# yshen47/SGAM_NeurIPS22

Measured on AMD Instinct MI355X. Metric: generated RGB-D frames/sec (256x256, GoogleEarth), higher is better.
Workload: dtype f32; 1 GPU; GoogleEarth-Infinite 256x256 inference loop (BASELINE configs[2]): forward-splat warp (N<=3) + VQGAN encode/quantise(4096)/decode + frame feedback, in-HBM frame store; frames_per_gpu=1105, scenes=1, parallelism=scene-parallel x1, launch=hip-graph replay of the VQGAN forward, f32_products=exact hi/lo fp16 split on the fp16 matrix cores, fp32 accumulate

## Files before the change

sgam_neurips22_amd/build.py:

```python
import hashlib
import os
import shutil
import subprocess
import sys

PKG = os.path.dirname(os.path.abspath(__file__))
CSRC = os.path.join(PKG, "csrc")
LIBDIR = os.environ.get("SGAM_LIB_DIR") or os.path.join(PKG, "lib")
LIB = os.path.join(LIBDIR, "libsgam_hip.so")
ARCH = "gfx950"

SOURCES = {
    "conv_gemm.hip": [],
    "norm_softmax.hip": [],
    "groupnorm.hip": [],
    "h16.hip": [],
    "conv_f32x.hip": [],
    "h16_halo.hip": [],
    "attention.hip": [],
    "vq.hip": ["-ffp-contract=off"],
    "layout.hip": ["-ffp-contract=off"],
    "warp.hip": ["-ffp-contract=off"],
    "gemm_gn_f32x.hip": [],
    "train.hip": [],
    "eval.hip": ["-ffp-contract=off"],
    "kmeans.hip": ["-ffp-contract=off"],
    "imageio.hip": ["-ffp-contract=off"],
    "build_info.hip": [],
    "tsdf.hip": ["-ffp-contract=off"],
    "mesh_raster.hip": ["-ffp-contract=off"],
    "point_raster.hip": ["-ffp-contract=off"],
    "point_nn.hip": ["-ffp-contract=off"],
    "point_cloud.hip": ["-ffp-contract=off"],
    "point_icp.hip": ["-ffp-contract=off"],
    "point_global.hip": ["-ffp-contract=off"],
    "mesh_ops.hip": ["-ffp-contract=off"],
    "mesh_query.hip": ["-ffp-contract=off"],
    "mesh_ray.hip": ["-ffp-contract=off"],
    "mesh_bvh.hip": ["-ffp-contract=off"],
    "inception.hip": ["-ffp-contract=off"],
    "feature_metrics.hip": ["-ffp-contract=off"],
}
COMMON = ["-O3", "-std=c++17", "-fPIC", f"--offload-arch={ARCH}", "-Wall", "-Wno-unused-function"]


def _hipcc():
    for cand in (os.environ.get("HIPCC"), shutil.which("hipcc"), "/opt/rocm/bin/hipcc"):
        if cand and os.path.exists(cand):
            return cand
    raise RuntimeError("hipcc not found: libsgam_hip.so cannot be built (ROCm toolchain required)")


def _git(*args):
    try:
        r = subprocess.run(["git", "-C", os.path.join(PKG, "..")] + list(args), capture_output=True, text=True, timeout=10)
        return r.stdout.strip() if r.returncode == 0 else None
    except (OSError, subprocess.SubprocessError):
        return None


_STAMP_PATHS = ["sgam_neurips22_amd/csrc", "include", "sgam_neurips22_amd/build.py"]


def build_stamp(headers):
    srcs = sorted(os.path.join(CSRC, f) for f in SOURCES if os.path.exists(os.path.join(CSRC, f)) and f != "build_info.hip")
    digest = _digest(srcs + headers, [COMMON] + [SOURCES[os.path.basename(p)] for p in srcs])[:12]
    stamp_file = os.path.join(LIBDIR, "BUILD_STAMP")
    commit = _git("log", "-1", "--format=%h", "--abbrev=12", "--", *_STAMP_PATHS)
    if commit:
        if _git("status", "--porcelain", "--", *_STAMP_PATHS):
            commit += "+dirty"
    else:
        commit = "nogit"
        if os.path.exists(stamp_file):
            old = open(stamp_file).read().split()
            if len(old) == 2 and old[1] == digest:
                commit = old[0]
    return commit, digest, stamp_file


def _digest(paths, flags):
    h = hashlib.sha256()
    for p in sorted(paths, key=os.path.basename):
        h.update(os.path.basename(p).encode())
        with open(p, "rb") as f:
            h.update(f.read())
    h.update(repr(flags).encode())
    return h.hexdigest()


def build(force=False, verbose=False):
    hipcc = _hipcc()
    os.makedirs(LIBDIR, exist_ok=True)
    headers = [os.path.join(CSRC, f) for f in os.listdir(CSRC) if f.endswith(".h")]
    headers.append(os.path.join(PKG, "..", "include", "sgam_hip.h"))
    objs, relink = [], force or not os.path.exists(LIB)
    commit, digest, stamp_file = build_stamp(headers)
    SOURCES["build_info.hip"] = [f'-DSGAM_BUILD_COMMIT="{commit}"', f'-DSGAM_BUILD_DIGEST="{digest}"']
    for src, extra in SOURCES.items():
        path = os.path.join(CSRC, src)
        if not os.path.exists(path):
            continue
        obj = os.path.join(LIBDIR, src.replace(".hip", ".o"))
        stamp = obj + ".sha"
        dig = _digest([path] + headers, COMMON + extra)
        old = open(stamp).read() if os.path.exists(stamp) else ""
        if force or not os.path.exists(obj) or old != dig:
            cmd = [hipcc] + COMMON + extra + ["-c", path, "-o", obj]
            if verbose:
                print(" ".join(cmd), flush=True)
            subprocess.check_call(cmd)
            with open(stamp, "w") as f:
                f.write(dig)
            relink = True
        objs.append(obj)
    if relink:
        cmd = [hipcc, "-shared", "-fPIC", f"--offload-arch={ARCH}", "-o", LIB] + objs
        if verbose:
            print(" ".join(cmd), flush=True)
        subprocess.check_call(cmd)
    with open(stamp_file, "w") as f:
        f.write(f"{commit} {digest}\n")
    return LIB


if __name__ == "__main__":
    print(build(force="--force" in sys.argv, verbose=True))
```

sgam_neurips22_amd/csrc/attention.hip:

```cpp
#include "sgam_common.h"

namespace {

typedef unsigned int u32x4 __attribute__((ext_vector_type(4)));
typedef unsigned int u32x2 __attribute__((ext_vector_type(2)));
typedef _Float16 f16x8 __attribute__((ext_vector_type(8)));

constexpr int AD = 256;
constexpr int KB = 32;
constexpr int BLK_BYTES = KB * AD * 4;
constexpr float P_LIFT = 10.0f;
constexpr float LOG2E = 1.4426950408889634f;
constexpr float RESCALE_TAU = 5.0f;

__device__ __forceinline__ f32x16 mfma16(u32x4 a, u32x4 b, f32x16 c) {
    return __builtin_amdgcn_mfma_f32_32x32x16_f16(__builtin_bit_cast(f16x8, a), __builtin_bit_cast(f16x8, b), c, 0, 0, 0);
}

__device__ __forceinline__ void split8(const float *v, u32x4 &hi, u32x4 &lo) {
#pragma unroll
    for (int e = 0; e < 4; ++e) {
        const _Float16 h0 = (_Float16)v[2 * e], h1 = (_Float16)v[2 * e + 1];
        const _Float16 l0 = (_Float16)(v[2 * e] - (float)h0), l1 = (_Float16)(v[2 * e + 1] - (float)h1);
        hi[e] = (unsigned)__builtin_bit_cast(unsigned short, h0) | ((unsigned)__builtin_bit_cast(unsigned short, h1) << 16);
        lo[e] = (unsigned)__builtin_bit_cast(unsigned short, l0) | ((unsigned)__builtin_bit_cast(unsigned short, l1) << 16);
    }
}

__global__ __launch_bounds__(256) void attn_split_kv_kernel(const float *__restrict__ k, const float *__restrict__ v, int ld,
                                                            int n, unsigned short *__restrict__ kf,
                                                            unsigned short *__restrict__ vf) {
    const int gid = blockIdx.x * 256 + threadIdx.x;
    const int row = gid & 31, h = (gid >> 5) & 1, t = (gid >> 6) & 1, tile = (gid >> 7) & 7, kb = gid >> 10;
    if (kb * KB >= n) return;
    float kv[8], vv[8];
    const float *kp = k + (int64_t)(kb * KB + row) * ld + tile * 32 + t * 16 + h * 8;
    const f32x4 k0 = *reinterpret_cast<const f32x4 *>(kp), k1 = *reinterpret_cast<const f32x4 *>(kp + 4);
#pragma unroll
    for (int e = 0; e < 4; ++e) {
        kv[e] = k0[e];
        kv[4 + e] = k1[e];
    }
#pragma unroll
    for (int s = 0; s < 8; ++s) {
        const int key = 4 * h + 8 * (2 * t + (s >> 2)) + (s & 3);
        vv[s] = v[(int64_t)(kb * KB + key) * ld + tile * 32 + row];
    }
    u32x4 hi, lo;
    const int64_t piece = ((int64_t)(kb * 8 + tile) * 256 + (t * 2 + h) * 32 + row) * 8;
    split8(kv, hi, lo);
    *reinterpret_cast<u32x4 *>(kf + piece) = hi;
    *reinterpret_cast<u32x4 *>(kf + piece + 128 * 8) = lo;
    split8(vv, hi, lo);
    *reinterpret_cast<u32x4 *>(vf + piece) = hi;
    *reinterpret_cast<u32x4 *>(vf + piece + 128 * 8) = lo;
}

struct AttnParams {
    const unsigned short *qf;
    const float *q;
    const unsigned short *kf, *vf;
    float *ws_o;
    float *ws_ml;
    int ld, n, blocks_per_split;
    int n_img, nsplit;
    float qscale;
};

constexpr int NSPLIT = 8;

typedef __attribute__((address_space(1))) const void gptr_t;
typedef __attribute__((address_space(3))) void lptr_t;

__global__ __launch_bounds__(256) void attn_flash_f32x_kernel(const AttnParams p) {
    __shared__ __attribute__((aligned(16))) unsigned char smem[4 * BLK_BYTES];
    const int tid = threadIdx.x, lane = tid & 63, wave = tid >> 6;
    const int sp = blockIdx.x % p.nsplit, qb = blockIdx.x / p.nsplit;
    const int q0 = qb * 128 + wave * 32;
    const int lq = lane & 31, lh = lane >> 5;
    const int kb0 = ((qb * 128) / p.n_img) * (p.n_img / KB) + sp * p.blocks_per_split, kb1 = kb0 + p.blocks_per_split;
    const unsigned char *kg = reinterpret_cast<const unsigned char *>(p.kf), *vg = reinterpret_cast<const unsigned char *>(p.vf);

    const int wave_s = __builtin_amdgcn_readfirstlane(wave);
    auto dma1 = [&](const unsigned char *g, int kb, int slot, const int i) {
        const unsigned char *src = g + (int64_t)kb * BLK_BYTES + wave_s * 8192 + (i >> 2) * 4096 + lane * 16;
        unsigned char *dst = smem + slot * BLK_BYTES + wave_s * 8192 + (i >> 2) * 4096;
        switch (i & 3) {
        case 0: __builtin_amdgcn_global_load_lds((gptr_t *)src, (lptr_t *)dst, 16, 0, 0); break;
        case 1: __builtin_amdgcn_global_load_lds((gptr_t *)src, (lptr_t *)dst, 16, 1024, 0); break;
        case 2: __builtin_amdgcn_global_load_lds((gptr_t *)src, (lptr_t *)dst, 16, 2048, 0); break;
        default: __builtin_amdgcn_global_load_lds((gptr_t *)src, (lptr_t *)dst, 16, 3072, 0); break;
        }
    };
    auto dma = [&](const unsigned char *g, int kb, int slot) {
#pragma unroll
        for (int i = 0; i < 8; ++i) dma1(g, kb, slot, i);
    };
    u32x4 qh[16], ql[16];
    if (p.qf) {
        const unsigned short *qb = p.qf + (int64_t)(q0 >> 5) * (16 * 1024) + lane * 8;
#pragma unroll
        for (int t = 0; t < 16; ++t) {
            qh[t] = *reinterpret_cast<const u32x4 *>(qb + t * 1024);
            ql[t] = *reinterpret_cast<const u32x4 *>(qb + t * 1024 + 512);
        }
    } else {
        const float *qp = p.q + (int64_t)(q0 + lq) * p.ld + lh * 8;
#pragma unroll
        for (int t = 0; t < 16; ++t) {
            const f32x4 a = *reinterpret_cast<const f32x4 *>(qp + t * 16), b = *reinterpret_cast<const f32x4 *>(qp + t * 16 + 4);
            float v[8];
#pragma unroll
            for (int e = 0; e < 4; ++e) {
                v[e] = a[e] * p.qscale;
                v[4 + e] = b[e] * p.qscale;
            }
            split8(v, qh[t], ql[t]);
        }
    }

    f32x16 o[8];
#pragma unroll
    for (int i = 0; i < 8; ++i)
#pragma unroll
        for (int e = 0; e < 16; ++e) o[i][e] = 0.f;
    float m_run = -INFINITY, l_run = 0.f;

    const int nb = kb1 - kb0;
    auto blk = [&](int j) { return kb0 + (j < nb ? j : nb - 1); };
    dma(kg, blk(0), 0);
    dma(vg, blk(0), 2);
    dma(kg, blk(1), 1);

    u32x4 fh[3], fl[3];
    f32x16 sacc[2];
    float s[16], pe[2];
    u32x4 ph[2], pl[2];
    auto lds_off = [](const unsigned char *ptr) {
        return (unsigned)(uintptr_t)(__attribute__((address_space(3))) const unsigned char *)ptr;
    };
#define ATTN_DS_READ(dst, addr, off) asm volatile("ds_read_b128 %0, %1 offset:%2" : "=v"(dst) : "v"(addr), "i"(off))
#define ATTN_DS_WAIT(n, set) asm volatile("s_waitcnt lgkmcnt(" #n ")" : "+v"(fh[set]), "+v"(fl[set]))
#define ATTN_BARRIER(cnt)                                        \
    do {                                                          \
        asm volatile("s_waitcnt vmcnt(" #cnt ")" ::: "memory");   \
        __builtin_amdgcn_s_barrier();                             \
    } while (0)
    auto smfma = [&](const int t) {
        sacc[(3 * t) & 1] = mfma16(fh[t % 3], qh[t], sacc[(3 * t) & 1]);
        sacc[(3 * t + 1) & 1] = mfma16(fh[t % 3], ql[t], sacc[(3 * t + 1) & 1]);
        sacc[(3 * t + 2) & 1] = mfma16(fl[t % 3], qh[t], sacc[(3 * t + 2) & 1]);
    };
#define ATTN_FRAG(set, base, t)                                              \
    do {                                                                      \
        ATTN_DS_READ(fh[set], base, ((t) >> 1) * 4096 + ((t) & 1) * 1024);        \
        ATTN_DS_READ(fl[set], base, ((t) >> 1) * 4096 + (2 + ((t) & 1)) * 1024);  \
    } while (0)
    ATTN_BARRIER(0);

    {
        const unsigned lk = lds_off(smem + lane * 16);
#pragma unroll
        for (int e = 0; e < 16; ++e) sacc[0][e] = sacc[1][e] = 0.f;
        ATTN_FRAG(0, lk, 0);
        ATTN_FRAG(1, lk, 1);
#pragma unroll
        for (int t = 0; t < 16; ++t) {
            if (t + 2 < 16) ATTN_FRAG((t + 2) % 3, lk, t + 2);
            if (t + 2 < 16) ATTN_DS_WAIT(4, t % 3);
            else if (t + 1 < 16) ATTN_DS_WAIT(2, t % 3);
            else ATTN_DS_WAIT(0, t % 3);
            smfma(t);
        }
        float mloc = -INFINITY;
#pragma unroll
        for (int e = 0; e < 16; ++e) {
            s[e] = (sacc[0][e] + sacc[1][e]) * LOG2E;
            mloc = fmaxf(mloc, s[e]);
        }
        m_run = fmaxf(mloc, __shfl_xor(mloc, 32, 64));
        ATTN_BARRIER(0);
        dma(kg, blk(2), 0);
    }

    for (int j = 0; j < nb; ++j) {
        const int buf = j & 1;
        const unsigned lk = lds_off(smem + (buf ^ 1) * BLK_BYTES + lane * 16);
        const unsigned lv = lds_off(smem + (2 + buf) * BLK_BYTES + lane * 16);
        const int kb_k = blk(j + 3), kb_v = blk(j + 1);
#pragma unroll
        for (int e = 0; e < 16; ++e) sacc[0][e] = sacc[1][e] = 0.f;
        ATTN_FRAG(0, lk, 0);
        ATTN_FRAG(1, lk, 1);
#pragma unroll
        for (int t = 0; t < 16; ++t) {
            if (t + 2 < 16) ATTN_FRAG((t + 2) % 3, lk, t + 2);
            if (t < 8) dma1(vg, kb_v, 2 + (buf ^ 1), t);
            if (t + 2 < 16) ATTN_DS_WAIT(4, t % 3);
            else if (t + 1 < 16) ATTN_DS_WAIT(2, t % 3);
            else ATTN_DS_WAIT(0, t % 3);
            smfma(t);
            pe[t & 1] = __builtin_amdgcn_exp2f(s[t] - m_run + P_LIFT);
            l_run += pe[t & 1];
            if (t & 1) {
                typedef _Float16 f16x2 __attribute__((ext_vector_type(2)));
                const f16x2 h = __builtin_bit_cast(f16x2, __builtin_amdgcn_cvt_pkrtz(pe[0], pe[1]));
                const f16x2 l = __builtin_bit_cast(f16x2, __builtin_amdgcn_cvt_pkrtz(pe[0] - (float)h[0], pe[1] - (float)h[1]));
                ph[t >> 3][(t & 7) >> 1] = __builtin_bit_cast(unsigned, h);
                pl[t >> 3][(t & 7) >> 1] = __builtin_bit_cast(unsigned, l);
            }
        }
        ATTN_BARRIER(16);
        float mloc = -INFINITY;
        ATTN_FRAG(16 % 3, lv, 0);
        ATTN_FRAG(17 % 3, lv, 1);
#pragma unroll
        for (int u = 0; u < 16; ++u) {
            if (u + 2 < 16) ATTN_FRAG((16 + u + 2) % 3, lv, u + 2);
            if (u < 8) dma1(kg, kb_k, buf ^ 1, u);
            if (u + 2 < 16) ATTN_DS_WAIT(4, (16 + u) % 3);
            else if (u + 1 < 16) ATTN_DS_WAIT(2, (16 + u) % 3);
            else ATTN_DS_WAIT(0, (16 + u) % 3);
            const int i = u >> 1, t = u & 1, set = (16 + u) % 3;
            o[i] = mfma16(fh[set], ph[t], o[i]);
            o[i] = mfma16(fh[set], pl[t], o[i]);
            o[i] = mfma16(fl[set], ph[t], o[i]);
            if (u >= 4) {
#pragma unroll
                for (int e = (u - 4) * 4 / 3; e < (u - 3) * 4 / 3; ++e) {
                    s[e] = (sacc[0][e] + sacc[1][e]) * LOG2E;
                    mloc = fmaxf(mloc, s[e]);
                }
            }
        }
        if (j + 1 < nb) {
            mloc = fmaxf(mloc, __shfl_xor(mloc, 32, 64));
            const float m_new = fmaxf(m_run, mloc);
            if (__any(m_new > m_run + RESCALE_TAU)) {
                const float alpha = __builtin_amdgcn_exp2f(m_run - m_new);
                l_run *= alpha;
#pragma unroll
                for (int i = 0; i < 8; ++i)
#pragma unroll
                    for (int e = 0; e < 16; ++e) {
                        float x = o[i][e], tmp;
                        asm volatile("v_accvgpr_read_b32 %1, %0\n\tv_mul_f32 %1, %1, %2\n\tv_accvgpr_write_b32 %0, %1"
                                     : "+a"(x), "=&v"(tmp)
                                     : "v"(alpha));
                        o[i][e] = x;
                    }
                m_run = m_new;
            }
        }
        ATTN_BARRIER(16);
    }
#undef ATTN_FRAG
#undef ATTN_BARRIER
#undef ATTN_DS_WAIT
#undef ATTN_DS_READ

    l_run += __shfl_xor(l_run, 32, 64);
    if (lh == 0) {
        float *ml = p.ws_ml + ((int64_t)sp * p.n + q0 + lq) * 2;
        ml[0] = m_run;
        ml[1] = l_run;
    }
    float *wo = p.ws_o + ((int64_t)sp * (p.n / 32) + (q0 >> 5)) * (AD * 32) + lq;
#pragma unroll
    for (int i = 0; i < 8; ++i)
#pragma unroll
        for (int e = 0; e < 16; ++e)
            wo[(32 * i + 8 * (e >> 2) + 4 * lh + (e & 3)) * 32] = o[i][e];
    asm volatile("s_waitcnt vmcnt(0)" ::: "memory");
}

template <int NS>
__global__ __launch_bounds__(256) void attn_combine_kernel(const float *__restrict__ ws_o, const float *__restrict__ ws_ml,
                                                           float *__restrict__ out, int ldo, int n, int32_t *range_flag) {
    __shared__ float tile[32][33];
    const int qt = blockIdx.x >> 3, dg = blockIdx.x & 7;
    const int q = threadIdx.x & 31, dsub = threadIdx.x >> 5;
    float w[NS], l[NS], o[NS][4], M = -INFINITY, L = 0.f;
#pragma unroll
    for (int s = 0; s < NS; ++s) {
        const float *ml = ws_ml + ((int64_t)s * n + qt * 32 + q) * 2;
        w[s] = ml[0];
        l[s] = ml[1];
    }
#pragma unroll
    for (int s = 0; s < NS; ++s)
#pragma unroll
        for (int j = 0; j < 4; ++j) o[s][j] = ws_o[(((int64_t)s * (n / 32) + qt) * AD + dg * 32 + dsub * 4 + j) * 32 + q];
#pragma unroll
    for (int s = 0; s < NS; ++s) M = fmaxf(M, w[s]);
#pragma unroll
    for (int s = 0; s < NS; ++s) {
        w[s] = __builtin_amdgcn_exp2f(w[s] - M);
        L += w[s] * l[s];
    }
    const float inv = 1.0f / L;
    float acc[4] = {0.f, 0.f, 0.f, 0.f};
#pragma unroll
    for (int s = 0; s < NS; ++s)
#pragma unroll
        for (int j = 0; j < 4; ++j) acc[j] += w[s] * o[s][j];
#pragma unroll
    for (int j = 0; j < 4; ++j) tile[q][dsub * 4 + j] = acc[j] * inv;
    __syncthreads();
    const int r = threadIdx.x >> 3, c4 = (threadIdx.x & 7) * 4;
    const f32x4 v = {tile[r][c4], tile[r][c4 + 1], tile[r][c4 + 2], tile[r][c4 + 3]};
    *reinterpret_cast<f32x4 *>(out + (int64_t)(qt * 32 + r) * ldo + dg * 32 + c4) = v;
    if (range_flag && sgam_not_finite((v[0] + v[1]) + (v[2] + v[3]))) atomicOr(range_flag, 1);
}

struct CombProjParams {
    const float *ws_o, *ws_ml;
    const unsigned short *w;
    const float *bias, *res;
    float *out;
    double *gn_partial;
    int n_img;
    int32_t *range_flag;
    int n, ns, ldr, ldc;
    float inv_w_scale;
};

template <int NS>
__global__ __launch_bounds__(256) void attn_combine_proj_f32x_kernel(const CombProjParams p) {
    constexpr int LDK = AD + 8;
    __shared__ __attribute__((aligned(16))) unsigned short sA[2][32][LDK];
    const int tid = threadIdx.x, lane = tid & 63, wave = tid >> 6;
    const int qt = blockIdx.x;
    const int lr = lane & 31, lh = lane >> 5;
    constexpr int WD = 4, KS = AD / 16, SLABS = AD / 32;
    const unsigned short *wt0 = p.w + (int64_t)(wave * 2) * SLABS * 2048, *wt1 = wt0 + (int64_t)SLABS * 2048;
    u32x4 wh[WD][2], wl[WD][2];
    auto wfrag = [&](int kstep, u32x4 (&hi)[2], u32x4 (&lo)[2]) {
        const int off = (kstep >> 1) * 2048 + (((kstep & 1) * 2 + lh) * 32 + lr) * 8;
        hi[0] = *reinterpret_cast<const u32x4 *>(wt0 + off);
        lo[0] = *reinterpret_cast<const u32x4 *>(wt0 + off + 1024);
        hi[1] = *reinterpret_cast<const u32x4 *>(wt1 + off);
        lo[1] = *reinterpret_cast<const u32x4 *>(wt1 + off + 1024);
    };
    const int q = tid & 31, dg = tid >> 5;
    float w[NS], l[NS], M = -INFINITY, L = 0.f;
#pragma unroll
    for (int s = 0; s < NS; ++s) {
        w[s] = p.ws_ml[((int64_t)s * p.n + qt * 32 + q) * 2];
        l[s] = p.ws_ml[((int64_t)s * p.n + qt * 32 + q) * 2 + 1];
    }
    const float *ob = p.ws_o + ((int64_t)qt * AD + dg * 32) * 32 + q;
    const int64_t sstride = (int64_t)p.n * AD;
    constexpr int CPS = NS >= 8 ? 16 : 32, NSTEP = 32 / CPS;
    for (int s = 0; s < NS; ++s) M = fmaxf(M, w[s]);
#pragma unroll
    for (int s = 0; s < NS; ++s) {
        w[s] = __builtin_amdgcn_exp2f(w[s] - M);
        L += w[s] * l[s];
    }
    const float inv = 1.0f / L;
    bool bad = false;
#pragma unroll
    for (int step = 0; step < NSTEP; ++step) {
        float cur[CPS][NS];
#pragma unroll
        for (int j = 0; j < CPS; ++j)
#pragma unroll
            for (int s = 0; s < NS; ++s) cur[j][s] = ob[s * sstride + (step * CPS + j) * 32];
        float a[CPS];
#pragma unroll
        for (int j = 0; j < CPS; ++j) a[j] = 0.f;
#pragma unroll
        for (int s = 0; s < NS; ++s)
#pragma unroll
            for (int j = 0; j < CPS; ++j) a[j] += w[s] * cur[j][s];
#pragma unroll
        for (int h4 = 0; h4 < CPS / 4; ++h4) {
            unsigned hi[2], lo[2];
#pragma unroll
            for (int e = 0; e < 2; ++e) {
                const float a0 = a[4 * h4 + 2 * e] * inv, a1 = a[4 * h4 + 2 * e + 1] * inv;
                bad |= sgam_not_finite(a0 + a1);
                const _Float16 h0 = (_Float16)a0, h1 = (_Float16)a1;
                const _Float16 l0 = (_Float16)(a0 - (float)h0), l1 = (_Float16)(a1 - (float)h1);
                hi[e] = (unsigned)__builtin_bit_cast(unsigned short, h0) | ((unsigned)__builtin_bit_cast(unsigned short, h1) << 16);
                lo[e] = (unsigned)__builtin_bit_cast(unsigned short, l0) | ((unsigned)__builtin_bit_cast(unsigned short, l1) << 16);
            }
            const int d = dg * 32 + step * CPS + 4 * h4;
            *reinterpret_cast<u32x2 *>(&sA[0][q][d]) = u32x2{hi[0], hi[1]};
            *reinterpret_cast<u32x2 *>(&sA[1][q][d]) = u32x2{lo[0], lo[1]};
        }
    }
    if (bad && p.range_flag) atomicOr(p.range_flag, 1);
#pragma unroll
    for (int t = 0; t < WD; ++t) wfrag(t, wh[t], wl[t]);
    const int m0 = qt * 32;
    float rres[2][16], rbias[2];
#pragma unroll
    for (int j = 0; j < 2; ++j) {
        const int nn = wave * 64 + j * 32 + lr;
        rbias[j] = p.bias ? p.bias[nn] : 0.f;
#pragma unroll
        for (int e = 0; e < 16; ++e) rres[j][e] = p.res ? p.res[(int64_t)(m0 + 8 * (e >> 2) + 4 * lh + (e & 3)) * p.ldr + nn] : 0.f;
    }
    __syncthreads();
    f32x16 acc[2];
#pragma unroll
    for (int j = 0; j < 2; ++j)
#pragma unroll
        for (int e = 0; e < 16; ++e) acc[j][e] = 0.f;
#pragma unroll
    for (int t = 0; t < KS; ++t) {
        u32x4 bh[2] = {wh[t % WD][0], wh[t % WD][1]}, bl[2] = {wl[t % WD][0], wl[t % WD][1]};
        wfrag(t + WD < KS ? t + WD : KS - 1, wh[t % WD], wl[t % WD]);
        __builtin_amdgcn_sched_barrier(0);
        const u32x4 ah = *reinterpret_cast<const u32x4 *>(&sA[0][lr][t * 16 + lh * 8]);
        const u32x4 al = *reinterpret_cast<const u32x4 *>(&sA[1][lr][t * 16 + lh * 8]);
#pragma unroll
        for (int j = 0; j < 2; ++j) {
            acc[j] = mfma16(ah, bh[j], acc[j]);
            acc[j] = mfma16(ah, bl[j], acc[j]);
            acc[j] = mfma16(al, bh[j], acc[j]);
        }
    }
#pragma unroll
    for (int j = 0; j < 2; ++j) {
// ... 850 lines not shown
    constexpr int QBYTES = 32 * LDQ * 2, PBYTES = NW * 4 * 16 * 64 * 4, KBYTES = 2 * (32 * NKT * NW) * (64 + 8) * 2;
    __shared__ __attribute__((aligned(16))) unsigned char smem[(QBYTES + KBYTES > PBYTES ? QBYTES + KBYTES : PBYTES)];
    __shared__ float red[2][NW][32];
    unsigned short *sQ = reinterpret_cast<unsigned short *>(smem);
    const int tid = threadIdx.x, lane = tid & 63, wave = tid >> 6;
    const int lr = lane & 31, lh = lane >> 5;
    const int q0 = blockIdx.x * 32, d0 = blockIdx.y * 128;
    const int kb = (q0 / p.n_img) * p.n_img + wave * (32 * NKT);
#pragma unroll
    for (int it = 0; it < 32 * (CD / 8) / NT; ++it) {
        const int idx = tid + NT * it, r = idx / (CD / 8), c8 = idx % (CD / 8);
        *reinterpret_cast<u32x4 *>(sQ + r * LDQ + 8 * c8) = *reinterpret_cast<const u32x4 *>(p.q + (int64_t)(q0 + r) * p.ld + 8 * c8);
    }
    f32x16 sacc[NKT];
#pragma unroll
    for (int i = 0; i < NKT; ++i)
#pragma unroll
        for (int e = 0; e < 16; ++e) sacc[i][e] = 0.f;
    constexpr int KEYS = 32 * NKT * NW, DCH = 64, NCH = CD / DCH, KLD = DCH + 8, PER = KEYS * (DCH / 8) / NT;
    static_assert(KEYS * (DCH / 8) % NT == 0, "whole 16-byte pieces per thread");
    unsigned short *sK = reinterpret_cast<unsigned short *>(smem + QBYTES);
    const unsigned short *kbase = p.k + (int64_t)((q0 / p.n_img) * p.n_img) * p.ld;
    u32x4 kr[PER];
    auto kfetch = [&](int c) {
#pragma unroll
        for (int i = 0; i < PER; ++i) {
            const int idx = tid + NT * i;
            kr[i] = *reinterpret_cast<const u32x4 *>(kbase + (int64_t)(idx / (DCH / 8)) * p.ld + c * DCH + 8 * (idx % (DCH / 8)));
        }
    };
    auto kstore = [&](int buf) {
#pragma unroll
        for (int i = 0; i < PER; ++i) {
            const int idx = tid + NT * i;
            *reinterpret_cast<u32x4 *>(sK + (buf * KEYS + idx / (DCH / 8)) * KLD + 8 * (idx % (DCH / 8))) = kr[i];
        }
    };
    kfetch(0);
    kstore(0);
    kfetch(1);
    __syncthreads();
#pragma unroll 1
    for (int c = 0; c < NCH; ++c) {
#pragma unroll
        for (int tt = 0; tt < DCH / 16; ++tt) {
            const int t = c * (DCH / 16) + tt;
            const u32x4 qf = *reinterpret_cast<const u32x4 *>(sQ + lr * LDQ + t * 16 + lh * 8);
#pragma unroll
            for (int i = 0; i < NKT; ++i)
                sacc[i] = HM<HT>::mfma(*reinterpret_cast<const u32x4 *>(sK + ((c & 1) * KEYS + wave * 32 * NKT + 32 * i + lr) * KLD + tt * 16 + lh * 8),
                                       qf, sacc[i]);
        }
        if (c + 1 < NCH) {
            kstore((c + 1) & 1);
            if (c + 2 < NCH) kfetch(c + 2);
        }
        __syncthreads();
    }
    unsigned short vv[4][NKT][2][8];
#pragma unroll
    for (int dt = 0; dt < 4; ++dt) {
        const unsigned short *vp = p.v + (int64_t)(kb + 4 * lh) * p.ld + d0 + dt * 32 + lr;
#pragma unroll
        for (int i = 0; i < NKT; ++i)
#pragma unroll
            for (int t = 0; t < 2; ++t)
#pragma unroll
                for (int sl = 0; sl < 8; ++sl) vv[dt][i][t][sl] = vp[(int64_t)(32 * i + 16 * t + 8 * (sl >> 2) + (sl & 3)) * p.ld];
    }
    __builtin_amdgcn_sched_barrier(0);
    float mx = -INFINITY;
#pragma unroll
    for (int i = 0; i < NKT; ++i)
#pragma unroll
        for (int e = 0; e < 16; ++e) {
            sacc[i][e] *= p.scale;
            mx = fmaxf(mx, sacc[i][e]);
        }
    mx = fmaxf(mx, __shfl_xor(mx, 32, 64));
    if (lh == 0) red[0][wave][lr] = mx;
    __syncthreads();
    mx = fmaxf(fmaxf(red[0][0][lr], red[0][1][lr]), fmaxf(red[0][2][lr], red[0][3][lr]));
    if constexpr (NW == 8) mx = fmaxf(mx, fmaxf(fmaxf(red[0][4][lr], red[0][5][lr]), fmaxf(red[0][6][lr], red[0][7][lr])));
    float sum = 0.f;
#pragma unroll
    for (int i = 0; i < NKT; ++i)
#pragma unroll
        for (int e = 0; e < 16; ++e) {
            sacc[i][e] = __expf(sacc[i][e] - mx);
            sum += sacc[i][e];
        }
    sum += __shfl_xor(sum, 32, 64);
    if (lh == 0) red[1][wave][lr] = sum;
    __syncthreads();
    float tot = (red[1][0][lr] + red[1][1][lr]) + (red[1][2][lr] + red[1][3][lr]);
    if constexpr (NW == 8) tot += (red[1][4][lr] + red[1][5][lr]) + (red[1][6][lr] + red[1][7][lr]);
    const float inv = 1.0f / tot;
    u32x4 pf[NKT][2];
#pragma unroll
    for (int i = 0; i < NKT; ++i)
#pragma unroll
        for (int t = 0; t < 2; ++t)
#pragma unroll
            for (int e = 0; e < 8; e += 2) pf[i][t][e >> 1] = HM<HT>::pack2(sacc[i][8 * t + e] * inv, sacc[i][8 * t + e + 1] * inv);
    float *part = reinterpret_cast<float *>(smem);
    __syncthreads();
    __builtin_amdgcn_sched_barrier(0);
#pragma unroll
    for (int dt = 0; dt < 4; ++dt) {
        f32x16 oacc;
#pragma unroll
        for (int e = 0; e < 16; ++e) oacc[e] = 0.f;
#pragma unroll
        for (int i = 0; i < NKT; ++i)
#pragma unroll
            for (int t = 0; t < 2; ++t) {
                u32x4 vf;
#pragma unroll
                for (int e = 0; e < 4; ++e) vf[e] = (unsigned)vv[dt][i][t][2 * e] | ((unsigned)vv[dt][i][t][2 * e + 1] << 16);
                oacc = HM<HT>::mfma(vf, pf[i][t], oacc);
            }
#pragma unroll
        for (int e = 0; e < 16; ++e) part[((wave * 4 + dt) * 16 + e) * 64 + lane] = oacc[e];
    }
    __syncthreads();
    {
        const int dt = wave & 3, j0 = (NW == 8) ? 2 * (wave >> 2) : 0;
        unsigned short *dst = p.out + (int64_t)(q0 + lr) * p.ldo + d0 + 32 * dt + 4 * lh;
#pragma unroll
        for (int jj = 0; jj < (NW == 8 ? 2 : 4); ++jj) {
            const int j = j0 + jj;
            float o[4];
#pragma unroll
            for (int r = 0; r < 4; ++r) {
                const int e = 4 * j + r;
                float a[NW];
#pragma unroll
                for (int w = 0; w < NW; ++w) a[w] = part[((w * 4 + dt) * 16 + e) * 64 + lane];
                o[r] = (a[0] + a[1]) + (a[2] + a[3]);
                if constexpr (NW == 8) o[r] += (a[4] + a[5]) + (a[6] + a[7]);
            }
            *reinterpret_cast<u32x2 *>(dst + 8 * j) = u32x2{HM<HT>::pack2(o[0], o[1]), HM<HT>::pack2(o[2], o[3])};
        }
    }
}

}

static int attn_nsplit(int n_img, int B) {
    int ns = NSPLIT;
    while (ns > 1 && (int64_t)(n_img / 128) * (ns / 2) * B >= 256 && (n_img / KB) % (ns / 2) == 0 && n_img / (ns / 2) <= 2048) ns /= 2;
    return ns;
}

extern "C" int64_t sgam_attention_f32x_batched_workspace_bytes(int32_t n, int32_t C, int32_t B) {
    if (C != AD || n < 256 || n % 256 != 0 || B < 1 || (int64_t)B * n >= (1 << 24)) return -1;
    const int64_t nsplit = attn_nsplit(n, B), nt = (int64_t)B * n;
    return 2 * nt * AD * 4 + nsplit * nt * AD * 4 + nsplit * nt * 2 * 4;
}

extern "C" int64_t sgam_attention_f32x_workspace_bytes(int32_t n, int32_t C) { return sgam_attention_f32x_batched_workspace_bytes(n, C, 1); }

extern "C" int sgam_attention_f32x_batched(const float *q, const float *k, const float *v, int32_t ld, int32_t n, int32_t C, int32_t B,
                                           float scale, float *out, int32_t ldo, void *workspace, int64_t workspace_bytes,
                                           void *stream) {
    if (!q || !k || !v || !out || !workspace) return SGAM_EINVAL;
    const int64_t need = sgam_attention_f32x_batched_workspace_bytes(n, C, B);
    if (need < 0 || ld < C || ld % 4 != 0 || ldo < C) return SGAM_EINVAL;
    int ex;
    if (!(scale > 0.f) || frexpf(scale, &ex) != 0.5f) return SGAM_EINVAL;
    if (workspace_bytes < need) return SGAM_EWORKSPACE;
    if (!sgam_aligned16(q) || !sgam_aligned16(k) || !sgam_aligned16(v) || !sgam_aligned16(workspace)) return SGAM_EALIGN;
    const int nsplit = attn_nsplit(n, B), nt = B * n;
    if ((n / KB) % nsplit != 0 || ldo % 4 != 0 || !sgam_aligned16(out)) return SGAM_EINVAL;
    hipStream_t s = sgam_stream(stream);
    unsigned short *kf = (unsigned short *)workspace;
    unsigned short *vf = kf + (int64_t)nt * AD * 2;
    float *ws_o = (float *)(vf + (int64_t)nt * AD * 2);
    float *ws_ml = ws_o + (int64_t)nsplit * nt * AD;
    SGAM_KLAUNCH(attn_split_kv_kernel, dim3(nt / KB * 8 * 128 / 256), dim3(256), 0, s, k, v, ld, nt, kf, vf);
    SGAM_LAUNCH_CHECK();
    AttnParams p;
    p.qf = nullptr; p.q = q; p.kf = kf; p.vf = vf; p.ws_o = ws_o; p.ws_ml = ws_ml;
    p.ld = ld; p.n = nt; p.n_img = n; p.nsplit = nsplit; p.blocks_per_split = n / KB / nsplit; p.qscale = scale;
    if (sgam_i_prof_on) sgam_i_prof_work(4.0 * B * n * (double)n * AD, 4.0 * 4.0 * nt * AD);
    SGAM_KLAUNCH(attn_flash_f32x_kernel, dim3(nt / 128 * nsplit), dim3(256), 0, s, p);
    SGAM_LAUNCH_CHECK();
    switch (nsplit) {
        case 8: SGAM_KLAUNCH(attn_combine_kernel<8>, dim3(nt / 32 * 8), dim3(256), 0, s, ws_o, ws_ml, out, ldo, nt, sgam_i_range_flag); break;
        case 4: SGAM_KLAUNCH(attn_combine_kernel<4>, dim3(nt / 32 * 8), dim3(256), 0, s, ws_o, ws_ml, out, ldo, nt, sgam_i_range_flag); break;
        case 2: SGAM_KLAUNCH(attn_combine_kernel<2>, dim3(nt / 32 * 8), dim3(256), 0, s, ws_o, ws_ml, out, ldo, nt, sgam_i_range_flag); break;
        case 1: SGAM_KLAUNCH(attn_combine_kernel<1>, dim3(nt / 32 * 8), dim3(256), 0, s, ws_o, ws_ml, out, ldo, nt, sgam_i_range_flag); break;
        default: return SGAM_EINVAL;
    }
    SGAM_LAUNCH_CHECK();
    return SGAM_OK;
}

extern "C" int sgam_attention_f32x(const float *q, const float *k, const float *v, int32_t ld, int32_t n, int32_t C,
                                   float scale, float *out, int32_t ldo, void *workspace, int64_t workspace_bytes,
                                   void *stream) {
    return sgam_attention_f32x_batched(q, k, v, ld, n, C, 1, scale, out, ldo, workspace, workspace_bytes, stream);
}

extern "C" int sgam_attention_proj_f32x_batched(const float *q, const float *k, const float *v, int32_t ld, int32_t n, int32_t C,
                                                int32_t B, float scale, const void *w_planes, float w_scale, const float *bias,
                                                const float *residual, int32_t ldr, float *out, int32_t ldc, double *gn_partial,
                                                void *workspace, int64_t workspace_bytes, void *stream) {
    if (!q || !k || !v || !out || !workspace || !w_planes || !(w_scale > 0.f)) return SGAM_EINVAL;
    const int64_t need = sgam_attention_f32x_batched_workspace_bytes(n, C, B);
    if (need < 0 || ld < C || ld % 4 != 0 || ldc < C || (residual && ldr < C)) return SGAM_EINVAL;
    int ex;
    if (!(scale > 0.f) || frexpf(scale, &ex) != 0.5f) return SGAM_EINVAL;
    if (workspace_bytes < need) return SGAM_EWORKSPACE;
    if (!sgam_aligned16(q) || !sgam_aligned16(k) || !sgam_aligned16(v) || !sgam_aligned16(workspace) || !sgam_aligned16(w_planes) ||
        (gn_partial && !sgam_aligned16(gn_partial)))
        return SGAM_EALIGN;
    const int nsplit = attn_nsplit(n, B), nt = B * n;
    if ((n / KB) % nsplit != 0) return SGAM_EINVAL;
    hipStream_t s = sgam_stream(stream);
    unsigned short *kf = (unsigned short *)workspace;
    unsigned short *vf = kf + (int64_t)nt * AD * 2;
    float *ws_o = (float *)(vf + (int64_t)nt * AD * 2);
    float *ws_ml = ws_o + (int64_t)nsplit * nt * AD;
    SGAM_KLAUNCH(attn_split_kv_kernel, dim3(nt / KB * 8 * 128 / 256), dim3(256), 0, s, k, v, ld, nt, kf, vf);
    SGAM_LAUNCH_CHECK();
    AttnParams p;
    p.qf = nullptr; p.q = q; p.kf = kf; p.vf = vf; p.ws_o = ws_o; p.ws_ml = ws_ml;
    p.ld = ld; p.n = nt; p.n_img = n; p.nsplit = nsplit; p.blocks_per_split = n / KB / nsplit; p.qscale = scale;
    if (sgam_i_prof_on) sgam_i_prof_work(4.0 * B * n * (double)n * AD, 4.0 * 4.0 * nt * AD);
    SGAM_KLAUNCH(attn_flash_f32x_kernel, dim3(nt / 128 * nsplit), dim3(256), 0, s, p);
    SGAM_LAUNCH_CHECK();
    CombProjParams c;
    c.ws_o = ws_o; c.ws_ml = ws_ml; c.w = (const unsigned short *)w_planes; c.bias = bias; c.res = residual; c.out = out;
    c.gn_partial = gn_partial; c.n_img = n;
    c.range_flag = sgam_i_range_flag; c.n = nt; c.ns = nsplit; c.ldr = ldr; c.ldc = ldc;
    c.inv_w_scale = 1.0f / w_scale;
    if (sgam_i_prof_on) sgam_i_prof_shape(nt, AD, AD, 1);
    if (sgam_i_prof_on) sgam_i_prof_work(2.0 * nt * (double)AD * AD, 4.0 * ((double)nsplit * nt * AD + 2.0 * nt * AD + (double)AD * AD));
    switch (nsplit) {
        case 8: SGAM_KLAUNCH(attn_combine_proj_f32x_kernel<8>, dim3(nt / 32), dim3(256), 0, s, c); break;
        case 4: SGAM_KLAUNCH(attn_combine_proj_f32x_kernel<4>, dim3(nt / 32), dim3(256), 0, s, c); break;
        case 2: SGAM_KLAUNCH(attn_combine_proj_f32x_kernel<2>, dim3(nt / 32), dim3(256), 0, s, c); break;
        case 1: SGAM_KLAUNCH(attn_combine_proj_f32x_kernel<1>, dim3(nt / 32), dim3(256), 0, s, c); break;
        default: return SGAM_EINVAL;
    }
    SGAM_LAUNCH_CHECK();
    return SGAM_OK;
}

extern "C" int64_t sgam_attention_h16_batched_workspace_bytes(int32_t n, int32_t C, int32_t B) {
    if (C != AD || n < 256 || n % 256 != 0 || B < 1 || (int64_t)B * n >= (1 << 24)) return -1;
    const int64_t nsplit = attn_nsplit(n, B), nt = (int64_t)B * n;
    return 2 * nt * AD * 2 + nsplit * nt * AD * 4 + nsplit * nt * 2 * 4;
}

extern "C" int64_t sgam_attention_h16_workspace_bytes(int32_t n, int32_t C) { return sgam_attention_h16_batched_workspace_bytes(n, C, 1); }

extern "C" int sgam_attention_h16_batched(const void *q, const void *k, const void *v, int32_t ht, int32_t ld, int32_t n, int32_t C,
                                          int32_t B, float scale, void *out, int32_t ldo, void *workspace, int64_t workspace_bytes,
                                          void *stream) {
    if (!q || !k || !v || !out || !workspace || (ht != 0 && ht != 1)) return SGAM_EINVAL;
    const int64_t need = sgam_attention_h16_batched_workspace_bytes(n, C, B);
    if (need < 0) return SGAM_EINVAL;
    const int nsplit = attn_nsplit(n, B), nt = B * n;
    if (ld < C || ld % 8 != 0 || ldo < C || ldo % 4 != 0 || !(scale > 0.f) || (n / KB) % nsplit != 0) return SGAM_EINVAL;
    if (workspace_bytes < need) return SGAM_EWORKSPACE;
    if (!sgam_aligned16(q) || !sgam_aligned16(k) || !sgam_aligned16(v) || !sgam_aligned16(workspace) ||
        (((uintptr_t)out) & 7u) != 0)
        return SGAM_EALIGN;
    hipStream_t s = sgam_stream(stream);
    unsigned short *kf = (unsigned short *)workspace;
    unsigned short *vf = kf + (int64_t)nt * AD;
    float *ws_o = (float *)(vf + (int64_t)nt * AD);
    float *ws_ml = ws_o + (int64_t)nsplit * nt * AD;
    SGAM_KLAUNCH(attn_split_kv_h16_kernel, dim3(nt / 8), dim3(256), 0, s, (const unsigned short *)k,
                       (const unsigned short *)v, ld, nt, kf, vf);
    SGAM_LAUNCH_CHECK();
    AttnHParams p;
    p.q_frag = 0; p.q = (const unsigned short *)q; p.kf = kf; p.vf = vf; p.ws_o = ws_o; p.ws_ml = ws_ml;
    p.ld = ld; p.n = nt; p.n_img = n; p.nsplit = nsplit; p.blocks_per_split = n / KB / nsplit; p.qscale_log2e = scale * LOG2E;
    const dim3 grid(nt / 128 * nsplit), cgrid(nt / 32 * 8);
    if (sgam_i_prof_on) sgam_i_prof_work(4.0 * B * n * (double)n * AD, 4.0 * 2.0 * nt * AD);
    if (ht == 0) SGAM_KLAUNCH(attn_flash_h16_kernel<0>, grid, dim3(256), 0, s, p);
    else SGAM_KLAUNCH(attn_flash_h16_kernel<1>, grid, dim3(256), 0, s, p);
    SGAM_LAUNCH_CHECK();
#define HCOMBINE(HT_, NS_) SGAM_KLAUNCH((attn_combine_h16_kernel<HT_, NS_>), cgrid, dim3(256), 0, s, ws_o, ws_ml, (unsigned short *)out, ldo, nt)
    switch (nsplit * 2 + (ht ? 1 : 0)) {
        case 16: HCOMBINE(0, 8); break;
        case 17: HCOMBINE(1, 8); break;
        case 8: HCOMBINE(0, 4); break;
        case 9: HCOMBINE(1, 4); break;
        case 4: HCOMBINE(0, 2); break;
        case 5: HCOMBINE(1, 2); break;
        case 2: HCOMBINE(0, 1); break;
        case 3: HCOMBINE(1, 1); break;
        default: return SGAM_EINVAL;
    }
#undef HCOMBINE
    SGAM_LAUNCH_CHECK();
    return SGAM_OK;
}

extern "C" int sgam_attention_h16(const void *q, const void *k, const void *v, int32_t ht, int32_t ld, int32_t n, int32_t C,
                                  float scale, void *out, int32_t ldo, void *workspace, int64_t workspace_bytes, void *stream) {
    return sgam_attention_h16_batched(q, k, v, ht, ld, n, C, 1, scale, out, ldo, workspace, workspace_bytes, stream);
// ... 249 lines not shown
```

Measured before the change: 419.1 frames/s.

## Specialise flash attention tail trips and add optional timestamp instrumentation

```diff
diff --git a/sgam_neurips22_amd/build.py b/sgam_neurips22_amd/build.py
--- a/sgam_neurips22_amd/build.py
+++ b/sgam_neurips22_amd/build.py
@@ -42,6 +42,8 @@
     "feature_metrics.hip": ["-ffp-contract=off"],
 }
 COMMON = ["-O3", "-std=c++17", "-fPIC", f"--offload-arch={ARCH}", "-Wall", "-Wno-unused-function"]
+if os.environ.get("SGAM_ATTN_STAMP") == "1" and os.environ.get("SGAM_LIB_DIR"):
+    SOURCES["attention.hip"] = ["-DSGAM_ATTN_STAMP"]
 
 
 def _hipcc():
diff --git a/sgam_neurips22_amd/csrc/attention.hip b/sgam_neurips22_amd/csrc/attention.hip
--- a/sgam_neurips22_amd/csrc/attention.hip
+++ b/sgam_neurips22_amd/csrc/attention.hip
@@ -72,9 +72,52 @@
 typedef __attribute__((address_space(1))) const void gptr_t;
 typedef __attribute__((address_space(3))) void lptr_t;
 
+constexpr int FLASH_S_PIECES[16] = {1, 1, 1, 1, 1, 1, 1, 1, 0, 0, 0, 0, 0, 0, 0, 0};
+constexpr int FLASH_PV_PIECES[16] = {1, 1, 1, 1, 1, 1, 1, 1, 0, 0, 0, 0, 0, 0, 0, 0};
+constexpr int flash_pieces_before(const int (&tab)[16], int step) {
+    int c = 0;
+    for (int i = 0; i < step; ++i) c += tab[i];
+    return c;
+}
+constexpr int FLASH_VS = flash_pieces_before(FLASH_S_PIECES, 16);
+static_assert(FLASH_VS <= 8 && FLASH_VS + flash_pieces_before(FLASH_PV_PIECES, 16) == 16, "8 pieces of V^T, then 8 of K, per trip");
+
+template <bool STAGE_V_, bool STAGE_K_, bool K_AHEAD_, bool LAST_>
+struct TripShape {
+    static constexpr bool STAGE_V = STAGE_V_, STAGE_K = STAGE_K_, K_AHEAD = K_AHEAD_, LAST = LAST_;
+    static constexpr int MID_CNT = (K_AHEAD ? 8 : 0) + (STAGE_V ? FLASH_VS : 0);
+    static constexpr int END_CNT = (STAGE_V ? 8 : 0) + (STAGE_K ? 8 : 0);
+};
+typedef TripShape<true, true, true, false> TripSteady;
+typedef TripShape<true, false, true, false> TripTail3;
+typedef TripShape<true, false, false, false> TripTail2;
+typedef TripShape<false, false, false, true> TripLast;
+
+#ifdef SGAM_ATTN_STAMP
+constexpr int FLASH_STAMP_SLOTS = 64;
+__device__ unsigned long long *attn_flash_stamp_buf;
+__device__ unsigned attn_flash_stamp_wgs;
+#define ATTN_STAMP64(dst)                                                                    \
+    do {                                                                                      \
+        __builtin_amdgcn_sched_barrier(0);                                                    \
+        asm volatile("s_memtime %0\n\ts_waitcnt lgkmcnt(0)" : "=s"(dst)::"memory");           \
+        __builtin_amdgcn_sched_barrier(0);                                                    \
+    } while (0)
+#define ATTN_REAL64(dst)                                                                     \
+    do {                                                                                      \
+        __builtin_amdgcn_sched_barrier(0);                                                    \
+        asm volatile("s_memrealtime %0\n\ts_waitcnt lgkmcnt(0)" : "=s"(dst)::"memory");       \
+        __builtin_amdgcn_sched_barrier(0);                                                    \
+    } while (0)
+#endif
+
 __global__ __launch_bounds__(256) void attn_flash_f32x_kernel(const AttnParams p) {
     __shared__ __attribute__((aligned(16))) unsigned char smem[4 * BLK_BYTES];
     const int tid = threadIdx.x, lane = tid & 63, wave = tid >> 6;
+#ifdef SGAM_ATTN_STAMP
+    unsigned long long st_entry, st_pro, st_end;
+    ATTN_STAMP64(st_entry);
+#endif
     const int sp = blockIdx.x % p.nsplit, qb = blockIdx.x / p.nsplit;
     const int q0 = qb * 128 + wave * 32;
     const int lq = lane & 31, lh = lane >> 5;
@@ -127,10 +170,9 @@
     float m_run = -INFINITY, l_run = 0.f;
 
     const int nb = kb1 - kb0;
-    auto blk = [&](int j) { return kb0 + (j < nb ? j : nb - 1); };
-    dma(kg, blk(0), 0);
-    dma(vg, blk(0), 2);
-    dma(kg, blk(1), 1);
+    dma(kg, kb0, 0);
+    dma(vg, kb0, 2);
+    if (nb > 1) dma(kg, kb0 + 1, 1);
 
     u32x4 fh[3], fl[3];
     f32x16 sacc[2];
@@ -141,10 +183,10 @@
     };
 #define ATTN_DS_READ(dst, addr, off) asm volatile("ds_read_b128 %0, %1 offset:%2" : "=v"(dst) : "v"(addr), "i"(off))
 #define ATTN_DS_WAIT(n, set) asm volatile("s_waitcnt lgkmcnt(" #n ")" : "+v"(fh[set]), "+v"(fl[set]))
-#define ATTN_BARRIER(cnt)                                        \
-    do {                                                          \
-        asm volatile("s_waitcnt vmcnt(" #cnt ")" ::: "memory");   \
-        __builtin_amdgcn_s_barrier();                             \
+#define ATTN_BARRIER(cnt)                                             \
+    do {                                                               \
+        asm volatile("s_waitcnt vmcnt(%0)" ::"n"(cnt) : "memory");     \
+        __builtin_amdgcn_s_barrier();                                  \
     } while (0)
     auto smfma = [&](const int t) {
         sacc[(3 * t) & 1] = mfma16(fh[t % 3], qh[t], sacc[(3 * t) & 1]);
@@ -157,6 +199,9 @@
         ATTN_DS_READ(fl[set], base, ((t) >> 1) * 4096 + (2 + ((t) & 1)) * 1024);  \
     } while (0)
     ATTN_BARRIER(0);
+#ifdef SGAM_ATTN_STAMP
+    ATTN_STAMP64(st_pro);
+#endif
 
     {
         const unsigned lk = lds_off(smem + lane * 16);
@@ -179,27 +224,69 @@
             mloc = fmaxf(mloc, s[e]);
         }
         m_run = fmaxf(mloc, __shfl_xor(mloc, 32, 64));
-        ATTN_BARRIER(0);
-        dma(kg, blk(2), 0);
-    }
-
-    for (int j = 0; j < nb; ++j) {
+        if (nb > 2) {
+            ATTN_BARRIER(0);
+            dma(kg, kb0 + 2, 0);
+        }
+    }
+#ifdef SGAM_ATTN_STAMP
+    unsigned long long st_loop0, st_loop1, st_real0, st_real1;
+    unsigned st_seg[35], st_trips = 0, st_rescales = 0;
+#pragma unroll
+    for (int i = 0; i < 35; ++i) st_seg[i] = 0;
+    ATTN_REAL64(st_real0);
+    ATTN_STAMP64(st_loop0);
+#endif
+
+    auto trip = [&](const int j, auto shape) {
+        typedef decltype(shape) SH;
+#ifdef SGAM_ATTN_STAMP
+        constexpr bool STAMPED = SH::STAGE_K;
+        unsigned long long st_prev = 0, st_now;
+        if constexpr (STAMPED) ATTN_STAMP64(st_prev);
+#define ATTN_STAMP_SEG(k)                                                       \
+    do {                                                                         \
+        if constexpr (STAMPED) {                                                 \
+            ATTN_STAMP64(st_now);                                                \
+            unsigned st_d;                                                       \
+            asm volatile("s_sub_u32 %1, %2, %3\n\tv_add_u32_e32 %0, %1, %0"      \
+                         : "+v"(st_seg[k]), "=&s"(st_d)                          \
+                         : "s"((unsigned)st_now), "s"((unsigned)st_prev)         \
+                         : "scc");                                               \
+            st_prev = st_now;                                                    \
+        }                                                                        \
+    } while (0)
+#else
+#define ATTN_STAMP_SEG(k) do { } while (0)
+#endif
         const int buf = j & 1;
         const unsigned lk = lds_off(smem + (buf ^ 1) * BLK_BYTES + lane * 16);
         const unsigned lv = lds_off(smem + (2 + buf) * BLK_BYTES + lane * 16);
-        const int kb_k = blk(j + 3), kb_v = blk(j + 1);
-#pragma unroll
-        for (int e = 0; e < 16; ++e) sacc[0][e] = sacc[1][e] = 0.f;
-        ATTN_FRAG(0, lk, 0);
-        ATTN_FRAG(1, lk, 1);
+        const int kb_k = kb0 + j + 3, kb_v = kb0 + j + 1;
+        auto piece = [&](const int pc) {
+            if (pc < 8) {
+                if constexpr (SH::STAGE_V) dma1(vg, kb_v, 2 + (buf ^ 1), pc);
+            } else {
+                if constexpr (SH::STAGE_K) dma1(kg, kb_k, buf ^ 1, pc - 8);
+            }
+        };
+        if constexpr (!SH::LAST) {
+#pragma unroll
+            for (int e = 0; e < 16; ++e) sacc[0][e] = sacc[1][e] = 0.f;
+            ATTN_FRAG(0, lk, 0);
+            ATTN_FRAG(1, lk, 1);
+        }
 #pragma unroll
         for (int t = 0; t < 16; ++t) {
-            if (t + 2 < 16) ATTN_FRAG((t + 2) % 3, lk, t + 2);
-            if (t < 8) dma1(vg, kb_v, 2 + (buf ^ 1), t);
-            if (t + 2 < 16) ATTN_DS_WAIT(4, t % 3);
-            else if (t + 1 < 16) ATTN_DS_WAIT(2, t % 3);
-            else ATTN_DS_WAIT(0, t % 3);
-            smfma(t);
+            if constexpr (!SH::LAST) {
+                if (t + 2 < 16) ATTN_FRAG((t + 2) % 3, lk, t + 2);
+#pragma unroll
+                for (int c = 0; c < FLASH_S_PIECES[t]; ++c) piece(flash_pieces_before(FLASH_S_PIECES, t) + c);
+                if (t + 2 < 16) ATTN_DS_WAIT(4, t % 3);
+                else if (t + 1 < 16) ATTN_DS_WAIT(2, t % 3);
+                else ATTN_DS_WAIT(0, t % 3);
+                smfma(t);
+            }
             pe[t & 1] = __builtin_amdgcn_exp2f(s[t] - m_run + P_LIFT);
             l_run += pe[t & 1];
             if (t & 1) {
@@ -209,15 +296,18 @@
                 ph[t >> 3][(t & 7) >> 1] = __builtin_bit_cast(unsigned, h);
                 pl[t >> 3][(t & 7) >> 1] = __builtin_bit_cast(unsigned, l);
             }
-        }
-        ATTN_BARRIER(16);
+            ATTN_STAMP_SEG(t);
+        }
+        ATTN_BARRIER(SH::MID_CNT);
+        ATTN_STAMP_SEG(16);
         float mloc = -INFINITY;
         ATTN_FRAG(16 % 3, lv, 0);
         ATTN_FRAG(17 % 3, lv, 1);
 #pragma unroll
         for (int u = 0; u < 16; ++u) {
             if (u + 2 < 16) ATTN_FRAG((16 + u + 2) % 3, lv, u + 2);
-            if (u < 8) dma1(kg, kb_k, buf ^ 1, u);
+#pragma unroll
+            for (int c = 0; c < FLASH_PV_PIECES[u]; ++c) piece(FLASH_VS + flash_pieces_before(FLASH_PV_PIECES, u) + c);
             if (u + 2 < 16) ATTN_DS_WAIT(4, (16 + u) % 3);
             else if (u + 1 < 16) ATTN_DS_WAIT(2, (16 + u) % 3);
             else ATTN_DS_WAIT(0, (16 + u) % 3);
@@ -225,15 +315,18 @@
             o[i] = mfma16(fh[set], ph[t], o[i]);
             o[i] = mfma16(fh[set], pl[t], o[i]);
             o[i] = mfma16(fl[set], ph[t], o[i]);
-            if (u >= 4) {
-#pragma unroll
-                for (int e = (u - 4) * 4 / 3; e < (u - 3) * 4 / 3; ++e) {
-                    s[e] = (sacc[0][e] + sacc[1][e]) * LOG2E;
-                    mloc = fmaxf(mloc, s[e]);
+            if constexpr (!SH::LAST) {
+                if (u >= 4) {
+#pragma unroll
+                    for (int e = (u - 4) * 4 / 3; e < (u - 3) * 4 / 3; ++e) {
+                        s[e] = (sacc[0][e] + sacc[1][e]) * LOG2E;
+                        mloc = fmaxf(mloc, s[e]);
+                    }
                 }
             }
-        }
-        if (j + 1 < nb) {
+            ATTN_STAMP_SEG(17 + u);
+        }
+        if constexpr (!SH::LAST) {
             mloc = fmaxf(mloc, __shfl_xor(mloc, 32, 64));
             const float m_new = fmaxf(m_run, mloc);
             if (__any(m_new > m_run + RESCALE_TAU)) {
@@ -250,10 +343,28 @@
                         o[i][e] = x;
                     }
                 m_run = m_new;
-            }
-        }
-        ATTN_BARRIER(16);
-    }
+#ifdef SGAM_ATTN_STAMP
+                ++st_rescales;
+#endif
+            }
+        }
+        ATTN_STAMP_SEG(33);
+        if constexpr (SH::K_AHEAD) ATTN_BARRIER(SH::END_CNT);
+        ATTN_STAMP_SEG(34);
+#ifdef SGAM_ATTN_STAMP
+        if constexpr (STAMPED) ++st_trips;
+#endif
+#undef ATTN_STAMP_SEG
+    };
+    int j = 0;
+    for (; j + 3 < nb; ++j) trip(j, TripSteady());
+    if (j + 2 < nb) trip(j++, TripTail3());
+    if (j + 1 < nb) trip(j++, TripTail2());
+    trip(j, TripLast());
+#ifdef SGAM_ATTN_STAMP
+    ATTN_STAMP64(st_loop1);
+    ATTN_REAL64(st_real1);
+#endif
 #undef ATTN_FRAG
 #undef ATTN_BARRIER
 #undef ATTN_DS_WAIT
@@ -272,6 +383,18 @@
         for (int e = 0; e < 16; ++e)
             wo[(32 * i + 8 * (e >> 2) + 4 * lh + (e & 3)) * 32] = o[i][e];
     asm volatile("s_waitcnt vmcnt(0)" ::: "memory");
+#ifdef SGAM_ATTN_STAMP
+    ATTN_STAMP64(st_end);
+    if (attn_flash_stamp_buf && blockIdx.x < attn_flash_stamp_wgs && lane == 0) {
+        unsigned long long *sb = attn_flash_stamp_buf + ((int64_t)blockIdx.x * 4 + wave) * FLASH_STAMP_SLOTS;
+        sb[0] = st_entry; sb[1] = st_pro; sb[2] = st_loop0; sb[3] = st_loop1; sb[4] = st_end; sb[5] = st_real0; sb[6] = st_real1;
+        sb[7] = st_trips;
+#pragma unroll
+        for (int i = 0; i < 35; ++i) sb[8 + i] = st_seg[i];
+        sb[43] += st_rescales;
+        sb[44] += nb - 1;
+    }
+#endif
 }
 
 template <int NS>
@@ -1428,6 +1551,22 @@
     while (ns > 1 && (int64_t)(n_img / 128) * (ns / 2) * B >= 256 && (n_img / KB) % (ns / 2) == 0 && n_img / (ns / 2) <= 2048) ns /= 2;
     return ns;
 }
+
+#ifdef SGAM_ATTN_STAMP
+extern "C" int sgam_attn_flash_stamp_buffer(void *buf, int32_t workgroups) {
+    unsigned long long *b = (unsigned long long *)buf;
+    const unsigned w = buf && workgroups > 0 ? (unsigned)workgroups : 0u;
+    if (hipDeviceSynchronize() != hipSuccess) return SGAM_EINVAL;
+    if (hipMemcpyToSymbol(HIP_SYMBOL(attn_flash_stamp_wgs), &w, sizeof(w)) != hipSuccess) return SGAM_EINVAL;
+    return hipMemcpyToSymbol(HIP_SYMBOL(attn_flash_stamp_buf), &b, sizeof(b)) == hipSuccess ? SGAM_OK : SGAM_EINVAL;
+}
+extern "C" void sgam_attn_flash_piece_table(int32_t *s_pieces, int32_t *pv_pieces) {
+    for (int i = 0; i < 16; ++i) {
+        s_pieces[i] = FLASH_S_PIECES[i];
+        pv_pieces[i] = FLASH_PV_PIECES[i];
+    }
+}
+#endif
 
 extern "C" int64_t sgam_attention_f32x_batched_workspace_bytes(int32_t n, int32_t C, int32_t B) {
     if (C != AD || n < 256 || n % 256 != 0 || B < 1 || (int64_t)B * n >= (1 << 24)) return -1;
```

Measured after the change: 419.1 frames/s. Within noise of the previous version (-0.0%).
